# PaddlePaddle/PaddleScience

Hardware: AMD Instinct MI355X
Metric: collocation-points/sec (PDE residual+grad) (higher is better)
Workload: dtype f32

## Files before the change

include/ppsci_hip.h:

```cpp
#ifndef PPSCI_HIP_H
#define PPSCI_HIP_H

#include <stddef.h>
#include <stdint.h>

#ifdef __cplusplus
extern "C" {
#endif

#define PPSCI_MAX_IN 8
#define PPSCI_MAX_DIRS 4
#define PPSCI_MAX_OUT 8
#define PPSCI_MAX_HIDDEN 16
#define PPSCI_MAX_PROG 128
#define PPSCI_MAX_RES 8
#define PPSCI_MAX_EPARAM 8
#define PPSCI_MAX_AUX 16

enum { PPSCI_OK = 0, PPSCI_E_INVALID = -1, PPSCI_E_UNSUPPORTED = -2, PPSCI_E_LAUNCH = -3 };
enum { PPSCI_ACT_TANH = 0, PPSCI_ACT_SILU = 1, PPSCI_ACT_SIN = 2, PPSCI_ACT_SIGMOID = 3, PPSCI_ACT_COS = 4, PPSCI_ACT_GELU = 5,
       PPSCI_ACT_SWISH = 6, PPSCI_ACT_STAN = 7,
       PPSCI_ACT_RELU = 8, PPSCI_ACT_LEAKY_RELU = 9, PPSCI_ACT_ELU = 10, PPSCI_ACT_SELU = 11, PPSCI_ACT_IDENTITY = 12 };
enum { PPSCI_EMBED_NONE = 0, PPSCI_EMBED_PERIOD = 1,
       PPSCI_EMBED_STREAMS = 2 };
// ... 115 lines not shown
int ppsci_causal_weights(int64_t n_points, int n_chunks, float tol, const float* value, const float* label,
                         const float* weight, const float* area, float* chunk_scratch, float* cw, void* stream);

int ppsci_taylor_bwd(const ppsci_mlp_desc* d, const float* params, int64_t n_points,
                     const float* const* inputs_host, const float* Ubar, const void* stash,
                     void* workspace, float* grad_partials, void* stream);
int ppsci_taylor_bwd_ws(const ppsci_mlp_desc* d, const float* params, int64_t n_points,
                        const float* const* inputs_host, const float* Ubar, const void* stash,
                        void* workspace, int64_t workspace_bytes, float* grad_partials, void* stream);

typedef struct ppsci_adam_args {
  float* m;
  float* v;
  float lr, beta1, beta2, eps, grad_scale;
  int64_t step_t;
} ppsci_adam_args;

int64_t ppsci_taylor_step_workspace_bytes(const ppsci_mlp_desc* d, const ppsci_epilogue_desc* e, int64_t n_points);
int ppsci_taylor_step_kind(const ppsci_mlp_desc* d, const ppsci_epilogue_desc* e, int64_t n_points);
void ppsci_set_fused_step(int on);
void ppsci_set_step_tail(int mode);
void ppsci_set_fast_program(int on);
void ppsci_set_static_program(int on);
int ppsci_epilogue_predecode(const ppsci_epilogue_desc* e, uint32_t* out256, int* n_loads);
typedef struct ppsci_step_plan ppsci_step_plan;
ppsci_step_plan* ppsci_taylor_step_plan(const ppsci_mlp_desc* d, const ppsci_epilogue_desc* e, float* params,
                                        int64_t n_points, const float* const* inputs_host, const float* const* aux_host,
                                        float* U, float* Ubar, float* residual_out, void* stash, void* workspace,
                                        int64_t workspace_bytes, float* loss_terms, float* grad);
int ppsci_taylor_step_run(ppsci_step_plan* plan, int accumulate, const ppsci_adam_args* adam, void* stream);
#define PPSCI_STEP_KEEP_FRAGMENTS 1
int ppsci_taylor_step_run_ex(ppsci_step_plan* plan, int accumulate, const ppsci_adam_args* adam, void* stream, int flags);
int ppsci_taylor_step_plan_apply(ppsci_step_plan* plan, const ppsci_adam_args* adam, void* stream);
int ppsci_taylor_step_plan_set_scales(ppsci_step_plan* plan, const ppsci_epilogue_desc* e);
int ppsci_taylor_step_run_main(ppsci_step_plan* plan, void* stream);
void ppsci_taylor_step_plan_free(ppsci_step_plan* plan);
int ppsci_taylor_step_plan_static(const ppsci_step_plan* plan, const char** name);
int ppsci_taylor_step(const ppsci_mlp_desc* d, const ppsci_epilogue_desc* e, float* params, int64_t n_points,
                      const float* const* inputs_host, const float* const* aux_host, float* U, float* Ubar,
                      float* residual_out, void* stash, void* workspace, int64_t workspace_bytes, float* loss_terms,
                      float* grad, int accumulate, const ppsci_adam_args* adam, void* stream);

int ppsci_reduce_rows(const float* partials, int64_t rows, int64_t cols, float* out, int accumulate,
                      void* stream);

int ppsci_adam_step(int64_t n, float* params, const float* grad, float* m, float* v, float lr,
                    float beta1, float beta2, float eps, int64_t step_t, float grad_scale,
                    void* stream);

#define PPSCI_OPT_SGD 0
#define PPSCI_OPT_MOMENTUM 1
#define PPSCI_OPT_RMSPROP 2
#define PPSCI_OPT_ADAMW 3
int ppsci_optim_step(int kind, int64_t n, float* params, const float* grad, float* state1, float* state2,
                     float* state3, const float* hyper, int flag, void* stream);

int ppsci_linear_materialize(int kind, int fin, int fout, const float* v, const float* g, const float* b, float* W,
                             float* b_out, void* stream);
int ppsci_linear_pullback(int kind, int fin, int fout, const float* v, const float* g, const float* gW,
                          const float* gb, float* gv, float* gg, float* gb_out, void* stream);
// ... 256 lines not shown
```

paddlescience_amd/_lib.py:

```python
from __future__ import annotations

import ctypes as C
import os
from typing import List, Optional, Sequence

MAX_IN, MAX_DIRS, MAX_OUT, MAX_HIDDEN, MAX_PROG, MAX_RES, MAX_AUX = 8, 4, 8, 16, 128, 8, 16

ACT = {"tanh": 0, "silu": 1, "sin": 2, "sigmoid": 3, "cos": 4, "gelu": 5, "swish": 6, "stan": 7, "relu": 8, "leaky_relu": 9,
       "elu": 10, "selu": 11, "identity": 12}
PARAM_ACTS = ("swish", "stan")
SIREN_W0 = 30.0
LINEAR_PLAIN, LINEAR_WEIGHT_NORM, LINEAR_RWF, LINEAR_FOURIER, LINEAR_BROADCAST = range(5)
LINEAR_PADDED = 100
EMBED_NONE, EMBED_PERIOD, EMBED_STREAMS = 0, 1, 2

(OP_LD_IN, OP_LD_U, OP_LD_AUX, OP_CONST, OP_ADD, OP_SUB, OP_MUL, OP_DIV, OP_NEG, OP_POW, OP_SIN, OP_COS,
 OP_TANH, OP_EXP, OP_LOG, OP_SQRT, OP_ABS, OP_SINH, OP_COSH, OP_TAN, OP_MAX, OP_MIN, OP_SIGN, OP_HEAVISIDE,
 OP_DETACH, OP_ASIN, OP_ACOS, OP_ATAN, OP_ATAN2, OP_ASINH, OP_ACOSH, OP_ATANH, OP_ERF, OP_LGAMMA, OP_CEIL, OP_FLOOR,
 OP_LD_PARAM, OP_COUNT) = range(38)
MAX_EPARAM = 8
STEP_KEEP_FRAGMENTS = 1


class MlpDesc(C.Structure):
# ... 112 lines not shown
    "ppsci_epilogue_losses": (C.c_int, [C.POINTER(EpilogueDesc), C.c_int64, C.POINTER(C.c_void_p), C.c_void_p,
                                        C.POINTER(C.c_void_p), C.c_void_p, C.c_void_p, C.c_void_p, C.c_void_p,
                                        C.c_void_p, C.c_void_p, C.c_void_p, C.c_void_p]),
    "ppsci_epilogue_params": (C.c_int, [C.POINTER(EpilogueDesc), C.c_int64, C.POINTER(C.c_void_p), C.c_void_p,
                                        C.POINTER(C.c_void_p), C.c_void_p, C.c_void_p, C.c_void_p, C.c_void_p,
                                        C.c_void_p, C.c_void_p]),
    "ppsci_taylor_bwd": (C.c_int, [C.POINTER(MlpDesc), C.c_void_p, C.c_int64, C.POINTER(C.c_void_p), C.c_void_p,
                                   C.c_void_p, C.c_void_p, C.c_void_p, C.c_void_p]),
    "ppsci_taylor_bwd_ws": (C.c_int, [C.POINTER(MlpDesc), C.c_void_p, C.c_int64, C.POINTER(C.c_void_p), C.c_void_p,
                                      C.c_void_p, C.c_void_p, C.c_int64, C.c_void_p, C.c_void_p]),
    "ppsci_dense_matvec": (C.c_int, [C.c_int64, C.c_int64, C.c_void_p, C.c_void_p, C.c_void_p, C.c_float, C.c_int, C.c_void_p,
                                     C.c_void_p]),
    "ppsci_csr_matvec": (C.c_int, [C.c_int64, C.c_int64, C.c_int64, C.c_void_p, C.c_void_p, C.c_void_p, C.c_void_p, C.c_void_p,
                                   C.c_float, C.c_void_p, C.c_void_p]),
    "ppsci_reduce_rows": (C.c_int, [C.c_void_p, C.c_int64, C.c_int64, C.c_void_p, C.c_int, C.c_void_p]),
    "ppsci_taylor_step_workspace_bytes": (C.c_int64, [C.POINTER(MlpDesc), C.POINTER(EpilogueDesc), C.c_int64]),
    "ppsci_taylor_step_kind": (C.c_int, [C.POINTER(MlpDesc), C.POINTER(EpilogueDesc), C.c_int64]),
    "ppsci_set_fused_step": (None, [C.c_int]),
    "ppsci_set_step_tail": (None, [C.c_int]),
    "ppsci_set_fast_program": (None, [C.c_int]),
    "ppsci_taylor_step_run_ex": (C.c_int, [C.c_void_p, C.c_int, C.POINTER(AdamArgs), C.c_void_p, C.c_int]),
    "ppsci_taylor_step_plan_apply": (C.c_int, [C.c_void_p, C.POINTER(AdamArgs), C.c_void_p]),
    "ppsci_set_static_program": (None, [C.c_int]),
    "ppsci_epilogue_predecode": (C.c_int, [C.POINTER(EpilogueDesc), C.POINTER(C.c_uint32), C.POINTER(C.c_int)]),
    "ppsci_taylor_step_plan_static": (C.c_int, [C.c_void_p, C.POINTER(C.c_char_p)]),
    "ppsci_taylor_step_plan": (C.c_void_p, [C.POINTER(MlpDesc), C.POINTER(EpilogueDesc), C.c_void_p, C.c_int64,
                                            C.POINTER(C.c_void_p), C.POINTER(C.c_void_p), C.c_void_p, C.c_void_p, C.c_void_p,
                                            C.c_void_p, C.c_void_p, C.c_int64, C.c_void_p, C.c_void_p]),
    "ppsci_taylor_step_run": (C.c_int, [C.c_void_p, C.c_int, C.POINTER(AdamArgs), C.c_void_p]),
    "ppsci_taylor_step_plan_set_scales": (C.c_int, [C.c_void_p, C.POINTER(EpilogueDesc)]),
    "ppsci_taylor_step_run_main": (C.c_int, [C.c_void_p, C.c_void_p]),
    "ppsci_taylor_step_plan_free": (None, [C.c_void_p]),
    "ppsci_taylor_step": (C.c_int, [C.POINTER(MlpDesc), C.POINTER(EpilogueDesc), C.c_void_p, C.c_int64, C.POINTER(C.c_void_p),
                                    C.POINTER(C.c_void_p), C.c_void_p, C.c_void_p, C.c_void_p, C.c_void_p, C.c_void_p,
                                    C.c_int64, C.c_void_p, C.c_void_p, C.c_int, C.POINTER(AdamArgs), C.c_void_p]),
    "ppsci_spectral_conv2d_fwd": (C.c_int, [C.POINTER(SpectralDesc), C.c_void_p, C.c_void_p, C.c_void_p, C.c_void_p,
                                            C.c_void_p]),
    "ppsci_spectral_conv2d_bwd": (C.c_int, [C.POINTER(SpectralDesc), C.c_void_p, C.c_void_p, C.c_void_p, C.c_void_p,
                                            C.c_void_p, C.c_void_p, C.c_void_p, C.c_void_p]),
    "ppsci_spectral_conv2d_bwd_real": (C.c_int, [C.POINTER(SpectralDesc), C.c_void_p, C.c_void_p, C.c_void_p, C.c_void_p,
                                                 C.c_void_p, C.c_void_p, C.c_void_p, C.c_float, C.c_int, C.c_void_p]),
    "ppsci_spectral_conv2d_fwd_scaled": (C.c_int, [C.POINTER(SpectralDesc), C.c_void_p, C.c_void_p, C.c_void_p, C.c_void_p,
                                                   C.c_float, C.c_int, C.c_void_p]),
    "ppsci_spectral_conv2d_bwd_real_scaled": (C.c_int, [C.POINTER(SpectralDesc), C.c_void_p, C.c_void_p, C.c_void_p,
                                                        C.c_void_p, C.c_void_p, C.c_void_p, C.c_void_p, C.c_float, C.c_int,
                                                        C.c_float, C.c_int, C.c_void_p]),
# ... 206 lines not shown
```

paddlescience_amd/csrc/ppsci_common.h:

```cpp
#pragma once

#include "ppsci_hip.h"

#ifdef PPSCI_EMU
#include "hip_emu.h"
#define PPSCI_LAUNCH(KERNEL, ARGT, grid, block, lds, stream, args)                                   \
  do {                                                                                               \
    ARGT _a = (args);                                                                                \
    emu::launch_named(#KERNEL, emu_dim3{(unsigned)(grid)}, emu_dim3{(unsigned)(block)}, (size_t)(lds), \
                      [](void* p) { KERNEL(*(ARGT*)p); }, &_a);                                      \
  } while (0)
#define PPSCI_SET_MAX_LDS(KERNEL, bytes) (0)
#define PPSCI_LAST_LAUNCH_ERROR() (0)
#define PPSCI_OCCUPANCY(KERNEL, block, lds, out) (*(out) = 2, 0)
#define __builtin_amdgcn_sched_barrier(x) ((void)0)
#define ppsci_block_sync_lds() __syncthreads()
#define ppsci_block_sync_mem() __syncthreads()
#define ppsci_acquire_agent() ((void)0)
#define ppsci_setprio(p) ((void)0)
#define PPSCI_OPAQUE(v) ((void)0)
static inline void ppsci_store_agent(float* p, float v) { *p = v; }
static inline void ppsci_store_agent4(f32x4* p, f32x4 v) { *p = v; }
static inline unsigned ppsci_readlane(unsigned v, int lane) {
  float f;
  std::memcpy(&f, &v, 4);
  const float* buf = emu::wave_publish(f);
  unsigned r;
  std::memcpy(&r, &buf[lane & 63], 4);
  return r;
}
#else
#include <hip/hip_runtime.h>
typedef float f32x4 __attribute__((ext_vector_type(4)));
typedef unsigned u32x2 __attribute__((ext_vector_type(2)));
typedef unsigned u32x4 __attribute__((ext_vector_type(4)));
#define PPSCI_DYN_SMEM(name) extern __shared__ __attribute__((aligned(16))) float name[]
#define PPSCI_OPAQUE(v) asm volatile("" : "+v"(v))
__device__ __forceinline__ unsigned ppsci_cvt_pk_bf16(float a, float b) {
// ... 135 lines not shown
```

paddlescience_amd/csrc/taylor_api.hip:

```cpp
#include "taylor_tile.h"
#include "taylor_step.h"
#include "epi_static.h"

#include <math.h>
#include <stdlib.h>
#include <string.h>

#include <mutex>

__global__ void __launch_bounds__(256) ppsci_presplit_kernel(const float* params, ppsci_derived q, int H, int L, int bwd,
                                                             u32x4* out) {
  const int NB = q.NB, NKP = NB / 2;
  const int per_layer = NB * NKP * 64;
  const int total = (L - 1) * per_layer;
  for (int idx = blockIdx.x * blockDim.x + threadIdx.x; idx < total; idx += gridDim.x * blockDim.x) {
    const int l = 1 + idx / per_layer, rem = idx % per_layer;
    const int lane = rem & 63, pair = rem >> 6, rb = pair / NKP, kp = pair - rb * NKP;
    const int g = lane >> 4, c = lane & 15;
    const float* W = params + q.offW[l];
    ppsci_split4 sp[2];
#pragma unroll
    for (int hlf = 0; hlf < 2; ++hlf) {
      const int kb = 2 * kp + hlf;
      f32x4 v;
// ... 280 lines not shown
extern "C" int ppsci_taylor_bwd_ws(const ppsci_mlp_desc* d, const float* params, int64_t n_points,
                                   const float* const* inputs_host, const float* Ubar, const void* stash,
                                   void* workspace, int64_t workspace_bytes, float* grad_partials, void* stream) {
  if (workspace_bytes < 0 || n_points <= 0 || !d)
    return taylor_bwd_impl(d, params, n_points, inputs_host, Ubar, stash, workspace, grad_partials, stream);
  const int knob = ppsci_get_bwd_layerwise();
  int64_t need = ppsci_bwd_workspace_bytes(d, n_points);
  if (need > 0 && need <= workspace_bytes)
    return taylor_bwd_impl(d, params, n_points, inputs_host, Ubar, stash, workspace, grad_partials, stream);
  ppsci_set_bwd_layerwise(!knob);
  const int64_t other = ppsci_bwd_workspace_bytes(d, n_points);
  int rc;
  if (other > 0 && other <= workspace_bytes) {
    rc = taylor_bwd_impl(d, params, n_points, inputs_host, Ubar, stash, workspace, grad_partials, stream);
  } else {
    ppsci_set_error("taylor_bwd: workspace of %lld bytes, %lld needed (ppsci_bwd_workspace_bytes)", (long long)workspace_bytes,
                    (long long)need);
    rc = PPSCI_E_INVALID;
  }
  ppsci_set_bwd_layerwise(knob);
  return rc;
}

static int g_fused_step = 1, g_step_tail = -1, g_fast_vm = 1, g_static_prog = 1;
extern "C" void ppsci_set_fast_program(int on) { g_fast_vm = on ? 1 : 0; }
extern "C" void ppsci_set_static_program(int on) { g_static_prog = on ? 1 : 0; }
extern "C" int ppsci_epilogue_predecode(const ppsci_epilogue_desc* e, uint32_t* out256, int* n_loads) {
  int nl = 0;
  if (!e || !out256) return -1;
  const int n = epi_fast_encode(*e, out256, &nl);
  if (n_loads) *n_loads = nl;
  return n;
}
extern "C" void ppsci_set_fused_step(int on) { g_fused_step = on ? 1 : 0; }
extern "C" void ppsci_set_step_tail(int mode) { g_step_tail = (mode < 0 || mode > 3) ? -1 : mode; }
#define PPSCI_FUSED_TREE_MAX_GRID 48

static int run_step_act(StepArgs& a, void* stream, int launch, int* grid) {
  if (a.f.d.fourier_half > 0) return PPSCI_E_UNSUPPORTED;
  if (launch == 2 ? a.t.fused != 0 : g_fused_step != 0) {
    int rc = PPSCI_E_UNSUPPORTED;
    const bool st = a.e.static_id > 0;
    switch (a.f.d.activation) {
      case PPSCI_ACT_TANH: rc = st ? ppsci_fused_static_run_tanh(a, stream, launch, grid) : ppsci_fused_run_tanh(a, stream, launch, grid); break;
      case PPSCI_ACT_SILU: rc = st ? ppsci_fused_static_run_silu(a, stream, launch, grid) : ppsci_fused_run_silu(a, stream, launch, grid); break;
      case PPSCI_ACT_SIN: rc = st ? ppsci_fused_static_run_sin(a, stream, launch, grid) : ppsci_fused_run_sin(a, stream, launch, grid); break;
      default: break;
    }
    if (rc != PPSCI_E_UNSUPPORTED || launch == 2) return rc;
    a.e.static_id = 0;
  }
  a.t.fused = 0;
  switch (a.f.d.activation) {
    case PPSCI_ACT_TANH: return ppsci_step_run_tanh(a, stream, launch, grid);
    case PPSCI_ACT_SILU: return ppsci_step_run_silu(a, stream, launch, grid);
    case PPSCI_ACT_SIN: return ppsci_step_run_sin(a, stream, launch, grid);
    default: ppsci_set_error("taylor_step: no one-launch kernel for activation %d", a.f.d.activation); return PPSCI_E_UNSUPPORTED;
  }
}

struct StepLayout {
  long long rows_w, rows_s, rows_l, tree, counters, frag, red_tmp, red_small, red_row, fastprog, total;
  int per_tile, psmall, rowlen, tree_rows;
};
// ... 193 lines not shown
  t.rows_w = ws + y.rows_w;
  t.rows_s = ws + y.rows_s;
  t.rows_l = ws + y.rows_l;
  t.tree = ws + y.tree;
  t.counters = (unsigned*)(ws + y.counters);
  t.grad = grad;
  t.loss_terms = loss_terms;
  t.p = params;
  t.per_tile = y.per_tile;
  t.psmall = y.psmall;
  t.n_res = e->n_res;
  t.rowlen = y.rowlen;
  return plan;
}

extern "C" void ppsci_taylor_step_plan_free(ppsci_step_plan* plan) { delete plan; }

extern "C" int ppsci_taylor_step_plan_static(const ppsci_step_plan* plan, const char** name) {
  const int id = plan ? plan->a.e.static_id : 0;
  if (name) *name = epi_static_name(id);
  return id;
}

extern "C" int ppsci_taylor_step_plan_set_scales(ppsci_step_plan* plan, const ppsci_epilogue_desc* e) {
  if (!plan || !e || e->n_res != plan->a.e.e.n_res) {
    ppsci_set_error("taylor_step_plan_set_scales: invalid argument");
    return PPSCI_E_INVALID;
  }
  for (int k = 0; k < e->n_res; ++k) plan->a.e.e.res[k].scale = e->res[k].scale;
  return PPSCI_OK;
}

extern "C" int ppsci_taylor_step_run(ppsci_step_plan* plan, int accumulate, const ppsci_adam_args* adam, void* stream) {
  return ppsci_taylor_step_run_ex(plan, accumulate, adam, stream, 0);
}

extern "C" int ppsci_taylor_step_run_ex(ppsci_step_plan* plan, int accumulate, const ppsci_adam_args* adam, void* stream, int flags) {
  if (!plan) {
    ppsci_set_error("taylor_step_run: invalid argument");
    return PPSCI_E_INVALID;
  }
  StepTail& t = plan->a.t;
  t.accumulate = accumulate ? 1 : 0;
  t.do_adam = 0;
  if (adam) {
    if (!adam->m || !adam->v || adam->step_t < 1) {
// ... 140 lines not shown
```

paddlescience_amd/csrc/taylor_fused.inc:

```
#include "taylor_tile.h"
#include "taylor_step_tail.h"
#include "epi_static.h"

#include <stdlib.h>
#include <string.h>
#include <type_traits>

#ifndef PPSCI_FUSED_STATIC
#define PPSCI_FUSED_STATIC 0
#endif
#define PPSCI_FUSED_EPI_SCRATCH ((PPSCI_MAX_RES + PPSCI_MAX_EPARAM) * 16)
#define PPSCI_FUSED_MAX_IN 4
#define PPSCI_FUSED_XJ(x, j) ((j) == 0 ? (x)[0] : ((j) == 1 ? (x)[1] : ((j) == 2 ? (x)[2] : (x)[3])))

#ifdef PPSCI_FUSED_TIMERS
#define PPSCI_FT(k)                                             \
  {                                                             \
    const unsigned long long now_ = __builtin_amdgcn_s_memtime(); \
    tacc[k] += now_ - tlast;                                    \
    tlast = now_;                                               \
  }
#else
#define PPSCI_FT(k)
#endif
// ... 12 lines not shown
}

#ifdef PPSCI_DBG_DUMP
__device__ float* ppsci_dbg_buf = nullptr;
extern "C" int ppsci_dbg_set(float* p) { return (int)hipMemcpyToSymbol(HIP_SYMBOL(ppsci_dbg_buf), &p, sizeof(p)); }
#define PPSCI_DBG_STRIDE 16384
#endif


static inline long long ppsci_fused_floats(const ppsci_mlp_desc& d, const ppsci_derived& q, int S, int n_instr) {
  const int m = d.d_out, pad4m = ((m + 3) / 4) * 4;
  long long fl = 2LL * ((q.d0 + d.n_hidden + m) * q.HP + pad4m);
  fl += (q.NB + 1) * m * S * PPSCI_TILE;
  fl += q.NB * d.d_raw * PPSCI_TILE;
  fl += (long long)q.NB * m * S * PPSCI_TILE;
  fl += PPSCI_FUSED_EPI_SCRATCH + PPSCI_MAX_RES * PPSCI_TILE;
  fl += 2LL * n_instr * PPSCI_TILE;
  fl += EPI_FAST_WORDS + PPSCI_MAX_RES + PPSCI_MAX_RES * PPSCI_TILE;
  fl += 2LL * S * q.NB * 3 * 64 * 2;
  fl += PPSCI_MAX_DIRS * q.HP;
  return fl;
}

template <int NB, int LH, int N1, int N2, int ACT, bool STATIC, int ABL = 0>
__global__ void __launch_bounds__(64 * NB, 2) taylor_fused_kernel(StepArgs args) {
  constexpr int S = 1 + N1 + N2;
  constexpr int HP = 16 * NB;
  constexpr int W = NB;
  constexpr int L = LH;
  constexpr int NKP = NB / 2;
  static_assert(NB == 4, "one feature block per wave, both k-pairs of a layer's fragments held in registers");
  PPSCI_DYN_SMEM(smem);
  const FwdArgs& a = args.f;
  const int tid = threadIdx.x, nthr = blockDim.x;
  const int lane = tid & 63, wave = __builtin_amdgcn_readfirstlane(tid >> 6);
  const int g = lane >> 4, c = lane & 15;
  const int H = a.d.width, m = a.d.d_out, d0 = a.q.d0, d_raw = a.d.d_raw;
  const int pad4m = ((m + 3) / 4) * 4;
  const int n_instr = args.e.e.n_instr;

  float* W0s = smem;
  float* Bs = W0s + d0 * HP;
  float* WLs = Bs + L * HP;
  float* BLs = WLs + m * HP;
  float* gW0 = BLs + pad4m;
  float* gB = gW0 + d0 * HP;
  float* gWL = gB + L * HP;
  float* gBL = gWL + m * HP;
  float* tin = gBL + pad4m;
// ... 407 lines not shown
        }
      }
    }
    }

    fetch_x(tile + (int)gridDim.x, xr);
    PPSCI_FT(6)
    f32x4 hb[S];
#pragma unroll
    for (int s = 0; s < S; ++s) hb[s] = (f32x4){0.f, 0.f, 0.f, 0.f};
    for (int cc = 0; cc < m; ++cc) {
      float ub[S];
#pragma unroll
      for (int s = 0; s < S; ++s) ub[s] = tinw[(cc * S + s) * PPSCI_TILE + c];
      const f32x4 w4 = *(const f32x4*)&WLs[cc * HP + 16 * wave + 4 * g];
#pragma unroll
      for (int s = 0; s < S; ++s) hb[s] += w4 * ub[s];
      if (wave == 0 && !PPSCI_ABL(2)) {
        const float sb = ppsci_row_sum16_last(ub[0]);
        if (lane == 15) atomicAdd(&gBL[cc], sb);
      }
    }

    auto bwd_layer = [&](auto lc) {
      constexpr int l = decltype(lc)::value;
      const float zs = ppsci_zscale(a.d, l);
      int lanel = lane;
      PPSCI_OPAQUE(lanel);
      const int g = lanel >> 4, c = lanel & 15;
      const int xcl = ppsci_xchunk(lanel >> 4, lanel & 15);
      const int xtl = ppsci_xchunk(lanel & 3, 4 * (lanel >> 4) + ((lanel & 15) >> 2));
      const u32x4* gf = (const u32x4*)args.b.xfrag + (long long)(l > 0 ? l - 1 : 0) * PPSCI_GFRAG_PER_LAYER(NB) + lanel;
      u32x4 Ab[NKP][3];
      {
        f32x4 D1, D2, D3, hv;
        if (PPSCI_ABL(7)) {
          hv = zst[l][0];
          D1 = (f32x4){0.5f, 0.5f, 0.5f, 0.5f}, D2 = (f32x4){0.1f, 0.1f, 0.1f, 0.1f}, D3 = (f32x4){0.01f, 0.01f, 0.01f, 0.01f};
        } else
          ppsci_act_from_stash4<ACT>(zst[l][0], hv, D1, D2, D3);
#ifdef PPSCI_DBG_DUMP
        if (ppsci_dbg_buf != nullptr && l == L - 1) {
          float* q = &ppsci_dbg_buf[(long long)blockIdx.x * PPSCI_DBG_STRIDE + 5120];
          *(f32x4*)&q[(0 * 256 + tid) * 4] = D2;
          *(f32x4*)&q[(1 * 256 + tid) * 4] = D3;
        }
#endif
        if constexpr (l == L - 1) {
          f32x4 hc[S];
          hc[0] = hv;
#pragma unroll
          for (int i = 0; i < N1; ++i) {
            hc[1 + i] = D1 * zst[l][1 + i];
            if (i < N2) hc[1 + N1 + i] = D2 * zst[l][1 + i] * zst[l][1 + i] + D1 * zst[l][1 + N1 + i];
          }
          for (int cc = 0; cc < (PPSCI_ABL(2) ? 0 : m); ++cc) {
            f32x4 t = (f32x4){0.f, 0.f, 0.f, 0.f};
// ... 16 lines not shown
          *(f32x4*)&q[(2 * 256 + tid) * 4] = D1;
        }
#endif
        {
          const f32x4 two = {2.f, 2.f, 2.f, 2.f};
          f32x4 accv = D1 * hb[0];
#pragma unroll
          for (int i = 0; i < N1; ++i) {
            const f32x4 zi = zst[l][1 + i];
            const f32x4 hbi = hb[1 + i];
            f32x4 zbi = D1 * hbi;
            accv += D2 * zi * hbi;
            if (i < N2) {
              const f32x4 zii = zst[l][1 + N1 + i];
              const f32x4 hb2 = hb[1 + N1 + i];
              hb[1 + N1 + i] = D1 * hb2;
              zbi += two * D2 * zi * hb2;
              accv += (D3 * zi * zi + D2 * zii) * hb2;
            }
            hb[1 + i] = zbi;
          }
          hb[0] = accv;
        }
        if (zs != 1.f) {
#pragma unroll
          for (int s = 0; s < S; ++s) hb[s] *= zs;
        }
#ifdef PPSCI_DBG_DUMP
        if (ppsci_dbg_buf != nullptr && l == L - 1) {
#pragma unroll
          for (int s = 0; s < S; ++s) *(f32x4*)&ppsci_dbg_buf[(long long)blockIdx.x * PPSCI_DBG_STRIDE + (s * 256 + tid) * 4] = hb[s];
        }
#endif
        if (!PPSCI_ABL(2)) {
          f32x4 sb4;
#pragma unroll
          for (int r = 0; r < 4; ++r) sb4[r] = ppsci_row_sum16_last(hb[0][r]);
#ifdef PPSCI_DBG_DUMP
          if (ppsci_dbg_buf != nullptr && l == L - 1) *(f32x4*)&ppsci_dbg_buf[(long long)blockIdx.x * PPSCI_DBG_STRIDE + 4096 + tid * 4] = sb4;
#endif
          if (c == 15) {
#pragma unroll
            for (int r = 0; r < 4; ++r) atomicAdd(&gB[l * HP + 16 * wave + 4 * g + r], sb4[r]);
          }
        }
        if constexpr (l > 0) {
          __builtin_amdgcn_sched_barrier(0);
#pragma unroll
          for (int kp = 0; kp < NKP; ++kp)
#pragma unroll
            for (int q = 0; q < 3; ++q) Ab[kp][q] = gf[((wave * NKP + kp) * 3 + q) * 64];
          __builtin_amdgcn_sched_barrier(0);
#pragma unroll
          for (int s = 0; s < S; ++s) {
            const ppsci_split4 sp = ppsci_fused_split<ABL>(hb[s]);
#pragma unroll
            for (int q = 0; q < 3; ++q)
              if (!PPSCI_ABL(9) || (sp.p[q][0] == 0x12345u && sp.p[q][1] == 0x54321u)) zx[ppsci_xpair(NB, s, wave, q, xcl)] = sp.p[q];
            __builtin_amdgcn_sched_barrier(0);
          }
        }
      }

      if constexpr (l > 0) {
        __builtin_amdgcn_sched_barrier(0);
        ppsci_block_sync_lds();
        PPSCI_FT(7)
#pragma unroll
        for (int s = 0; s < S; ++s) hb[s] = (f32x4){0.f, 0.f, 0.f, 0.f};
        {
          u32x4 bq[2][S];
          const auto load_b = [&](int grp, u32x4 (&dst)[S]) {
            const int kp = grp / 3, pb = 2 - grp % 3;
#pragma unroll
            for (int s = 0; s < S; ++s) dst[s] = *(const u32x4*)&zx[ppsci_xpair(NB, s, 2 * kp, pb, xcl)];
          };
          load_b(0, bq[0]);
#pragma unroll
          for (int grp = 0; grp < 3 * NKP; ++grp) {
            const int kp = grp / 3, pb = 2 - grp % 3;
            if (grp + 1 < 3 * NKP) load_b(grp + 1, bq[(grp + 1) & 1]);
// ... 23 lines not shown
          f32x4 hcs[S];
          if (PPSCI_ABL(7)) {
            hcs[0] = zst[l - 1][0];
            E1 = (f32x4){0.5f, 0.5f, 0.5f, 0.5f}, E2 = (f32x4){0.1f, 0.1f, 0.1f, 0.1f};
          } else
            ppsci_act_from_stash4<ACT>(zst[l - 1][0], hcs[0], E1, E2, E3);
#pragma unroll
          for (int i = 0; i < N1; ++i) {
            hcs[1 + i] = E1 * zst[l - 1][1 + i];
            if (i < N2) hcs[1 + N1 + i] = E2 * zst[l - 1][1 + i] * zst[l - 1][1 + i] + E1 * zst[l - 1][1 + N1 + i];
          }
#pragma unroll
          for (int s = 0; s < S; ++s) {
            const ppsci_split4 sp = ppsci_fused_split<ABL>(hcs[s]);
#pragma unroll
            for (int q = 0; q < 3; ++q)
              if (!PPSCI_ABL(9) || (sp.p[q][0] == 0x12345u && sp.p[q][1] == 0x54321u)) hx[((s * NB + wave) * 3 + q) * 64 + xcl] = sp.p[q];
            __builtin_amdgcn_sched_barrier(0);
          }
        }
        __builtin_amdgcn_sched_barrier(0);
        if (!PPSCI_ABL(3)) ppsci_block_sync_lds();
        PPSCI_FT(9)
#pragma unroll 1
        for (int sp = 0; sp + 1 < (PPSCI_ABL(3) ? 0 : S); sp += 2) {
          int zs_ = ppsci_xpair(NB, sp, wave, 0, xtl);
          int hs_ = HPAIR ? ppsci_xpair(NB, sp, 0, 0, xtl) : xtl + sp * NB * 3 * 64;
          PPSCI_OPAQUE(zs_);
          PPSCI_OPAQUE(hs_);
          u32x2 zN0[3], zN1[3];
#pragma unroll
          for (int q = 0; q < 3; ++q) {
            zN0[q] = ppsci_lds_read_tr16(&zx[zs_ + q * 128]);
            zN1[q] = ppsci_lds_read_tr16(&zx[zs_ + (NKP * 3 + q) * 128]);
          }
          constexpr int IG = 2;
          u32x2 hN0[2][IG][3], hN1[2][IG][3];
          const auto load_h = [&](int ig, int buf) {
#pragma unroll
            for (int e = 0; e < IG; ++e)
#pragma unroll
              for (int q = 0; q < 3; ++q) {
                if constexpr (HPAIR) {
                  hN0[buf][e][q] = ppsci_lds_read_tr16(&hx[hs_ + (((ig + e) >> 1) * 3 + q) * 128 + ((ig + e) & 1)]);
                  hN1[buf][e][q] = ppsci_lds_read_tr16(&hx[hs_ + ((NKP + ((ig + e) >> 1)) * 3 + q) * 128 + ((ig + e) & 1)]);
                } else {
// ... 143 lines not shown
    const int k = idx / H, f = idx - k * H;
    ppsci_store_agent(&prow[idx], gW0[k * HP + f]);
  }
  for (int idx = tid; idx < L * H; idx += nthr) {
    const int l = idx / H, f = idx - l * H;
    ppsci_store_agent(&prow[d0 * H + idx], gB[l * HP + f]);
  }
  for (int idx = tid; idx < H * m; idx += nthr) {
    const int f = idx / m, cc = idx - f * m;
    ppsci_store_agent(&prow[(d0 + L) * H + idx], gWL[cc * HP + f]);
  }
  for (int idx = tid; idx < m; idx += nthr) ppsci_store_agent(&prow[(d0 + L + m) * H + idx], gBL[idx]);
  {
    float lsum[PPSCI_MAX_RES], padj[PPSCI_MAX_EPARAM];
#pragma unroll
    for (int k = 0; k < PPSCI_MAX_RES; ++k) lsum[k] = (wave == 0 && lane < PPSCI_TILE) ? lacc[k * PPSCI_TILE + lane] : 0.f;
#pragma unroll
    for (int k = 0; k < PPSCI_MAX_EPARAM; ++k) padj[k] = 0.f;
    epi_finale<EPI_RF_FUSED>(args.e, ered, lsum, padj);
  }
  if (args.t.external != 1) ppsci_step_tail(args.t, args.b.d, args.b.q, smem);
}

template <int NB, int LH, int N1, int N2>
static int launch_fused(StepArgs& a, void* stream, int launch, int* grid_out) {
  constexpr int S = 1 + N1 + N2;
  if (launch == 2) {
#ifdef PPSCI_ABL_BUILD
    {
      const char* ev = getenv("PPSCI_ABL");
      const int mask = ev ? atoi(ev) : 0;
#define PPSCI_ABL_CASE(M_)                                                                                                          \
  if (mask == (M_)) {                                                                                                               \
    PPSCI_SET_MAX_LDS((taylor_fused_kernel<NB, LH, N1, N2, PPSCI_ACT_ID, PPSCI_FUSED_STATIC != 0, (M_)>), a.t.lds);                    \
    PPSCI_LAUNCH((taylor_fused_kernel<NB, LH, N1, N2, PPSCI_ACT_ID, PPSCI_FUSED_STATIC != 0, (M_)>), StepArgs, a.t.grid, 64 * NB, a.t.lds, \
                 stream, a);                                                                                                        \
    return PPSCI_LAST_LAUNCH_ERROR() != 0 ? PPSCI_E_LAUNCH : PPSCI_OK;                                                              \
  }
      PPSCI_ABL_CASE(1) PPSCI_ABL_CASE(2) PPSCI_ABL_CASE(4) PPSCI_ABL_CASE(8) PPSCI_ABL_CASE(16) PPSCI_ABL_CASE(32) PPSCI_ABL_CASE(64)
      PPSCI_ABL_CASE(128) PPSCI_ABL_CASE(256) PPSCI_ABL_CASE(512)
#undef PPSCI_ABL_CASE
    }
#endif
    PPSCI_LAUNCH((taylor_fused_kernel<NB, LH, N1, N2, PPSCI_ACT_ID, PPSCI_FUSED_STATIC != 0>), StepArgs, a.t.grid, 64 * NB, a.t.lds, stream, a);
    int e = PPSCI_LAST_LAUNCH_ERROR();
    if (e != 0) {
      ppsci_set_error("taylor_fused: launch failed (hip error %d)", e);
      return PPSCI_E_LAUNCH;
    }
    return PPSCI_OK;
  }
  const long long fl = ppsci_fused_floats(a.f.d, a.f.q, S, a.e.e.n_instr);
  if (fl * 4 > PPSCI_LDS_LIMIT_BYTES / 2) {
    ppsci_set_error("taylor_fused: LDS need %lld B exceeds half a CU", fl * 4);
    return PPSCI_E_UNSUPPORTED;
  }
  const int lds = (int)(fl * 4);
  if (PPSCI_SET_MAX_LDS((taylor_fused_kernel<NB, LH, N1, N2, PPSCI_ACT_ID, PPSCI_FUSED_STATIC != 0>), lds) != 0) {
    ppsci_set_error("taylor_fused: cannot raise dynamic LDS to %d B", lds);
    return PPSCI_E_LAUNCH;
  }
  int per_cu = 1;
  if (PPSCI_OCCUPANCY((taylor_fused_kernel<NB, LH, N1, N2, PPSCI_ACT_ID, PPSCI_FUSED_STATIC != 0>), 64 * NB, lds, &per_cu) != 0 || per_cu < 1) per_cu = 1;
  const int ntl = a.f.ntiles;
  int grid = ntl < PPSCI_NUM_CU * per_cu ? ntl : PPSCI_NUM_CU * per_cu;
  if (ppsci_get_max_grid() > 0 && grid > ppsci_get_max_grid()) grid = ppsci_get_max_grid();
  if (grid < 1) grid = 1;
  a.f.iters = a.b.iters = a.e.iters = (ntl + grid - 1) / grid;
  a.f.tile0 = a.b.tile0 = 0;
  a.f.resident = a.b.resident = 1;
  a.b.accum = 1;
  a.b.xdl_split = 1;
  a.t.grid = grid;
  a.t.lds = lds;
  a.t.fused = 1;
  if (grid_out) *grid_out = grid;
  if (!launch) return PPSCI_OK;
  PPSCI_LAUNCH((taylor_fused_kernel<NB, LH, N1, N2, PPSCI_ACT_ID, PPSCI_FUSED_STATIC != 0>), StepArgs, grid, 64 * NB, lds, stream, a);
  int e = PPSCI_LAST_LAUNCH_ERROR();
  if (e != 0) {
    ppsci_set_error("taylor_fused: launch failed (hip error %d)", e);
    return PPSCI_E_LAUNCH;
  }
  return PPSCI_OK;
}

template <int N1, int N2, class... Ps>
static constexpr bool fused_has_static(epi_typelist<Ps...>) {
  return (false || ... || (Ps::N1 == N1 && Ps::N2 == N2));
}

template <int NB, int N1, int N2>
static int run_fused(StepArgs& a, void* stream, int launch, int* grid_out) {
  if constexpr (PPSCI_FUSED_STATIC != 0 && !fused_has_static<N1, N2>(EpiStaticPrograms{})) return PPSCI_E_UNSUPPORTED;
  else
  switch (a.f.d.n_hidden) {
    case 2: return launch_fused<NB, 2, N1, N2>(a, stream, launch, grid_out);
    case 3: return launch_fused<NB, 3, N1, N2>(a, stream, launch, grid_out);
    case 4: return launch_fused<NB, 4, N1, N2>(a, stream, launch, grid_out);
    case 5: return launch_fused<NB, 5, N1, N2>(a, stream, launch, grid_out);
    default: return PPSCI_E_UNSUPPORTED;
  }
}

int PPSCI_FUSED_RUN_NAME(StepArgs& a, void* stream, int launch, int* grid_out) {
#define PPSCI_FUSED_CASE(NB_, N1_, N2_) \
  if (a.f.q.NB == NB_ && a.f.d.n1 == N1_ && a.f.d.n2 == N2_ && a.f.d.n3 == 0) return run_fused<NB_, N1_, N2_>(a, stream, launch, grid_out);
// ... 10 lines not shown
```

paddlescience_amd/csrc/taylor_step.h:

```cpp
#pragma once
#include "epilogue_vm.h"

#ifdef PPSCI_EMU
#define PPSCI_STEP_FAN 3
#else
#define PPSCI_STEP_FAN 16
#endif

struct StepTail {
  float* rows_w;
  float* rows_s;
  float* rows_l;
  float* tree;
  unsigned* counters;
  float* grad;
  float* loss_terms;
  float* p;
  float* m;
  float* v;
  int grid, per_tile, psmall, n_res, rowlen;
  int lds;
  int accumulate, do_adam;
  float lr_t, beta1, beta2, eps_t, grad_scale;
  int fused;
  int one_tail;
  int external;
};

struct StepArgs {
  FwdArgs f;
  BwdArgs b;
  EpiArgs e;
  StepTail t;
};

int ppsci_step_run_tanh(StepArgs& a, void* stream, int launch, int* grid_out);
int ppsci_step_run_silu(StepArgs& a, void* stream, int launch, int* grid_out);
int ppsci_step_run_sin(StepArgs& a, void* stream, int launch, int* grid_out);
int ppsci_fused_run_tanh(StepArgs& a, void* stream, int launch, int* grid_out);
int ppsci_fused_run_silu(StepArgs& a, void* stream, int launch, int* grid_out);
int ppsci_fused_run_sin(StepArgs& a, void* stream, int launch, int* grid_out);
int ppsci_fused_static_run_tanh(StepArgs& a, void* stream, int launch, int* grid_out);
int ppsci_fused_static_run_silu(StepArgs& a, void* stream, int launch, int* grid_out);
int ppsci_fused_static_run_sin(StepArgs& a, void* stream, int launch, int* grid_out);
```

paddlescience_amd/hotpath.py:

```python
from __future__ import annotations

import ctypes as C
from dataclasses import dataclass, field
from typing import Dict, List, Optional, Sequence, Tuple

import torch

from . import _lib as L


def _stream_ptr(t: torch.Tensor):
    if t.is_cuda:
        return C.c_void_p(torch._C._cuda_getCurrentRawStream(t.device.index))
    return None


def _p(t: Optional[torch.Tensor]):
    return None if t is None else C.c_void_p(t.data_ptr())


def _chk_f32(*ts):
    for t in ts:
        if t is not None and (t.dtype != torch.float32 or not t.is_contiguous()):
            raise ValueError("hot-path buffers must be contiguous float32 tensors")
# ... 169 lines not shown
            aa = C.byref(L.AdamArgs(adam["m"].data_ptr(), adam["v"].data_ptr(), adam["lr"], adam["beta1"], adam["beta2"],
                                    adam["eps"], adam.get("grad_scale", 1.0), adam["t"]))
        capturing = self._params.is_cuda and torch.cuda.is_current_stream_capturing()
        keep = (not capturing and self._frag_token is not None
                and self._frag_token == (_PARAM_WRITES[0], self._params._version))
        L.check(self._run(self.handle, 1 if accumulate else 0, aa, _stream_ptr(self._dev), L.STEP_KEEP_FRAGMENTS if keep else 0))
        if adam is not None:
            note_param_write()
        self._frag_token = None if capturing else (_PARAM_WRITES[0], self._params._version)

    def apply_adam(self, adam: dict) -> None:
        aa = L.AdamArgs(adam["m"].data_ptr(), adam["v"].data_ptr(), adam["lr"], adam["beta1"], adam["beta2"], adam["eps"],
                        adam.get("grad_scale", 1.0), adam["t"])
        L.check(L.lib().ppsci_taylor_step_plan_apply(self.handle, C.byref(aa), _stream_ptr(self._dev)))
        note_param_write()
        capturing = self._params.is_cuda and torch.cuda.is_current_stream_capturing()
        self._frag_token = None if capturing else (_PARAM_WRITES[0], self._params._version)

    @property
    def static_program(self) -> str:
        nm = C.c_char_p()
        return (nm.value or b"").decode() if L.lib().ppsci_taylor_step_plan_static(self.handle, C.byref(nm)) > 0 else ""

    def run_main(self) -> None:
        L.check(L.lib().ppsci_taylor_step_run_main(self.handle, _stream_ptr(self._dev)))

    def __del__(self):
        h, self.handle = getattr(self, "handle", None), None
        if h:
            self._free(h)


_PARAM_WRITES = [0]


def note_param_write() -> None:
    _PARAM_WRITES[0] += 1


def dense_matvec(M: torch.Tensor, x: torch.Tensor, y: torch.Tensor, alpha: float = 1.0, transpose: bool = False,
                 rowscale: Optional[torch.Tensor] = None) -> None:
    _require_device(y)
    _chk_f32(M, x, y, rowscale)
    rows, cols = M.shape
    assert x.numel() >= (rows if transpose else cols) and y.numel() >= (cols if transpose else rows)
    L.check(L.lib().ppsci_dense_matvec(rows, cols, _p(M), _p(x), _p(rowscale), float(alpha), 1 if transpose else 0, _p(y),
# ... 181 lines not shown
```

Baseline: 445.1 million.

## Interleave next layer's pointwise adjoint with weight-gradient MFMAs in fused backward

Adds an OVL variant of the fused Taylor step kernel for static tanh programs with four streams and up to four hidden layers. In the reverse sweep, the pointwise adjoint, scaling, bias reduction, fragment load and LDS publish for layer l-1 are interleaved with the weight-gradient MFMA sweep of layer l. sched_group_barrier hints alternate matrix and VALU instructions. The aim is to hide VALU and LDS latency behind matrix-core work. The cost is higher register pressure from the carried fragment buffer, which could reduce occupancy, and a larger code footprint. It is on by default when the shape matches, with a setter and a plan query added.

```diff
diff --git a/include/ppsci_hip.h b/include/ppsci_hip.h
--- a/include/ppsci_hip.h
+++ b/include/ppsci_hip.h
@@ -161,6 +161,7 @@
 void ppsci_set_step_tail(int mode);
 void ppsci_set_fast_program(int on);
 void ppsci_set_static_program(int on);
+void ppsci_set_fused_overlap(int on);
 int ppsci_epilogue_predecode(const ppsci_epilogue_desc* e, uint32_t* out256, int* n_loads);
 typedef struct ppsci_step_plan ppsci_step_plan;
 ppsci_step_plan* ppsci_taylor_step_plan(const ppsci_mlp_desc* d, const ppsci_epilogue_desc* e, float* params,
@@ -175,6 +176,7 @@
 int ppsci_taylor_step_run_main(ppsci_step_plan* plan, void* stream);
 void ppsci_taylor_step_plan_free(ppsci_step_plan* plan);
 int ppsci_taylor_step_plan_static(const ppsci_step_plan* plan, const char** name);
+int ppsci_taylor_step_plan_overlap(const ppsci_step_plan* plan);
 int ppsci_taylor_step(const ppsci_mlp_desc* d, const ppsci_epilogue_desc* e, float* params, int64_t n_points,
                       const float* const* inputs_host, const float* const* aux_host, float* U, float* Ubar,
                       float* residual_out, void* stash, void* workspace, int64_t workspace_bytes, float* loss_terms,
diff --git a/paddlescience_amd/_lib.py b/paddlescience_amd/_lib.py
--- a/paddlescience_amd/_lib.py
+++ b/paddlescience_amd/_lib.py
@@ -158,6 +158,8 @@
     "ppsci_taylor_step_run_ex": (C.c_int, [C.c_void_p, C.c_int, C.POINTER(AdamArgs), C.c_void_p, C.c_int]),
     "ppsci_taylor_step_plan_apply": (C.c_int, [C.c_void_p, C.POINTER(AdamArgs), C.c_void_p]),
     "ppsci_set_static_program": (None, [C.c_int]),
+    "ppsci_set_fused_overlap": (None, [C.c_int]),
+    "ppsci_taylor_step_plan_overlap": (C.c_int, [C.c_void_p]),
     "ppsci_epilogue_predecode": (C.c_int, [C.POINTER(EpilogueDesc), C.POINTER(C.c_uint32), C.POINTER(C.c_int)]),
     "ppsci_taylor_step_plan_static": (C.c_int, [C.c_void_p, C.POINTER(C.c_char_p)]),
     "ppsci_taylor_step_plan": (C.c_void_p, [C.POINTER(MlpDesc), C.POINTER(EpilogueDesc), C.c_void_p, C.c_int64,
diff --git a/paddlescience_amd/csrc/ppsci_common.h b/paddlescience_amd/csrc/ppsci_common.h
--- a/paddlescience_amd/csrc/ppsci_common.h
+++ b/paddlescience_amd/csrc/ppsci_common.h
@@ -14,6 +14,7 @@
 #define PPSCI_LAST_LAUNCH_ERROR() (0)
 #define PPSCI_OCCUPANCY(KERNEL, block, lds, out) (*(out) = 2, 0)
 #define __builtin_amdgcn_sched_barrier(x) ((void)0)
+#define __builtin_amdgcn_sched_group_barrier(mask, n, id) ((void)0)
 #define ppsci_block_sync_lds() __syncthreads()
 #define ppsci_block_sync_mem() __syncthreads()
 #define ppsci_acquire_agent() ((void)0)
diff --git a/paddlescience_amd/csrc/taylor_api.hip b/paddlescience_amd/csrc/taylor_api.hip
--- a/paddlescience_amd/csrc/taylor_api.hip
+++ b/paddlescience_amd/csrc/taylor_api.hip
@@ -326,7 +326,8 @@
   return rc;
 }
 
-static int g_fused_step = 1, g_step_tail = -1, g_fast_vm = 1, g_static_prog = 1;
+static int g_fused_step = 1, g_step_tail = -1, g_fast_vm = 1, g_static_prog = 1, g_fused_overlap = 1;
+extern "C" void ppsci_set_fused_overlap(int on) { g_fused_overlap = on ? 1 : 0; }
 extern "C" void ppsci_set_fast_program(int on) { g_fast_vm = on ? 1 : 0; }
 extern "C" void ppsci_set_static_program(int on) { g_static_prog = on ? 1 : 0; }
 extern "C" int ppsci_epilogue_predecode(const ppsci_epilogue_desc* e, uint32_t* out256, int* n_loads) {
@@ -344,6 +345,7 @@
   if (a.f.d.fourier_half > 0) return PPSCI_E_UNSUPPORTED;
   if (launch == 2 ? a.t.fused != 0 : g_fused_step != 0) {
     int rc = PPSCI_E_UNSUPPORTED;
+    if (launch != 2) a.t.overlap = g_fused_overlap;
     const bool st = a.e.static_id > 0;
     switch (a.f.d.activation) {
       case PPSCI_ACT_TANH: rc = st ? ppsci_fused_static_run_tanh(a, stream, launch, grid) : ppsci_fused_run_tanh(a, stream, launch, grid); break;
@@ -583,6 +585,8 @@
   return id;
 }
 
+extern "C" int ppsci_taylor_step_plan_overlap(const ppsci_step_plan* plan) { return plan && plan->a.t.fused ? plan->a.t.overlap : 0; }
+
 extern "C" int ppsci_taylor_step_plan_set_scales(ppsci_step_plan* plan, const ppsci_epilogue_desc* e) {
   if (!plan || !e || e->n_res != plan->a.e.e.n_res) {
     ppsci_set_error("taylor_step_plan_set_scales: invalid argument");
diff --git a/paddlescience_amd/csrc/taylor_fused.inc b/paddlescience_amd/csrc/taylor_fused.inc
--- a/paddlescience_amd/csrc/taylor_fused.inc
+++ b/paddlescience_amd/csrc/taylor_fused.inc
@@ -58,9 +58,12 @@
   return fl;
 }
 
-template <int NB, int LH, int N1, int N2, int ACT, bool STATIC, int ABL = 0>
+#define PPSCI_FUSED_OVL_OK(LH_, N1_, N2_, STATIC_, ACT_) \
+  ((STATIC_) && (ACT_) == PPSCI_ACT_TANH && (N1_) == 2 && (N2_) == 1 && (LH_) <= 4)
+template <int NB, int LH, int N1, int N2, int ACT, bool STATIC, int ABL = 0, bool OVL = false>
 __global__ void __launch_bounds__(64 * NB, 2) taylor_fused_kernel(StepArgs args) {
   constexpr int S = 1 + N1 + N2;
+  static_assert(!OVL || (PPSCI_FUSED_OVL_OK(LH, N1, N2, STATIC, ACT) && ABL == 0), "the interleaved reverse sweep is written for S = 4, L <= 4");
   constexpr int HP = 16 * NB;
   constexpr int W = NB;
   constexpr int L = LH;
@@ -514,6 +517,7 @@
       }
     }
 
+    u32x4 AbT[NKP][3];
     auto bwd_layer = [&](auto lc) {
       constexpr int l = decltype(lc)::value;
       const float zs = ppsci_zscale(a.d, l);
@@ -523,8 +527,11 @@
       const int xcl = ppsci_xchunk(lanel >> 4, lanel & 15);
       const int xtl = ppsci_xchunk(lanel & 3, 4 * (lanel >> 4) + ((lanel & 15) >> 2));
       const u32x4* gf = (const u32x4*)args.b.xfrag + (long long)(l > 0 ? l - 1 : 0) * PPSCI_GFRAG_PER_LAYER(NB) + lanel;
-      u32x4 Ab[NKP][3];
-      {
+      constexpr bool PW_DONE = OVL && l < L - 1;
+      u32x4 AbL[NKP][3];
+      u32x4(&Ab)[NKP][3] = *(PW_DONE ? &AbT : &AbL);
+      const auto pw_adjoint = [&](auto kc) {
+        constexpr int l = decltype(kc)::value;
         f32x4 D1, D2, D3, hv;
         if (PPSCI_ABL(7)) {
           hv = zst[l][0];
@@ -587,6 +594,9 @@
           }
           hb[0] = accv;
         }
+      };
+      const auto pw_scale = [&](auto kc, const float zs) {
+        constexpr int l = decltype(kc)::value;
         if (zs != 1.f) {
 #pragma unroll
           for (int s = 0; s < S; ++s) hb[s] *= zs;
@@ -597,31 +607,47 @@
           for (int s = 0; s < S; ++s) *(f32x4*)&ppsci_dbg_buf[(long long)blockIdx.x * PPSCI_DBG_STRIDE + (s * 256 + tid) * 4] = hb[s];
         }
 #endif
-        if (!PPSCI_ABL(2)) {
-          f32x4 sb4;
-#pragma unroll
-          for (int r = 0; r < 4; ++r) sb4[r] = ppsci_row_sum16_last(hb[0][r]);
+      };
+      const auto pw_bias_sum = [&](auto kc) {
+        constexpr int l = decltype(kc)::value;
+        f32x4 sb4;
+#pragma unroll
+        for (int r = 0; r < 4; ++r) sb4[r] = ppsci_row_sum16_last(hb[0][r]);
 #ifdef PPSCI_DBG_DUMP
-          if (ppsci_dbg_buf != nullptr && l == L - 1) *(f32x4*)&ppsci_dbg_buf[(long long)blockIdx.x * PPSCI_DBG_STRIDE + 4096 + tid * 4] = sb4;
-#endif
-          if (c == 15) {
-#pragma unroll
-            for (int r = 0; r < 4; ++r) atomicAdd(&gB[l * HP + 16 * wave + 4 * g + r], sb4[r]);
-          }
-        }
+        if (ppsci_dbg_buf != nullptr && l == L - 1) *(f32x4*)&ppsci_dbg_buf[(long long)blockIdx.x * PPSCI_DBG_STRIDE + 4096 + tid * 4] = sb4;
+#endif
+        return sb4;
+      };
+      const auto pw_bias_add = [&](auto kc, const f32x4 sb4) {
+        constexpr int l = decltype(kc)::value;
+        if (c == 15) {
+#pragma unroll
+          for (int r = 0; r < 4; ++r) atomicAdd(&gB[l * HP + 16 * wave + 4 * g + r], sb4[r]);
+        }
+      };
+      const auto pw_frag = [&](const u32x4* gf, u32x4(&dst)[NKP][3]) {
+#pragma unroll
+        for (int kp = 0; kp < NKP; ++kp)
+#pragma unroll
+          for (int q = 0; q < 3; ++q) dst[kp][q] = gf[((wave * NKP + kp) * 3 + q) * 64];
+      };
+      const auto pw_publish = [&](int s) {
+        const ppsci_split4 sp = ppsci_fused_split<ABL>(hb[s]);
+#pragma unroll
+        for (int q = 0; q < 3; ++q)
+          if (!PPSCI_ABL(9) || (sp.p[q][0] == 0x12345u && sp.p[q][1] == 0x54321u)) zx[ppsci_xpair(NB, s, wave, q, xcl)] = sp.p[q];
+      };
+      if constexpr (!PW_DONE) {
+        pw_adjoint(lc);
+        pw_scale(lc, zs);
+        if (!PPSCI_ABL(2)) pw_bias_add(lc, pw_bias_sum(lc));
         if constexpr (l > 0) {
           __builtin_amdgcn_sched_barrier(0);
-#pragma unroll
-          for (int kp = 0; kp < NKP; ++kp)
-#pragma unroll
-            for (int q = 0; q < 3; ++q) Ab[kp][q] = gf[((wave * NKP + kp) * 3 + q) * 64];
+          pw_frag(gf, Ab);
           __builtin_amdgcn_sched_barrier(0);
 #pragma unroll
           for (int s = 0; s < S; ++s) {
-            const ppsci_split4 sp = ppsci_fused_split<ABL>(hb[s]);
-#pragma unroll
-            for (int q = 0; q < 3; ++q)
-              if (!PPSCI_ABL(9) || (sp.p[q][0] == 0x12345u && sp.p[q][1] == 0x54321u)) zx[ppsci_xpair(NB, s, wave, q, xcl)] = sp.p[q];
+            pw_publish(s);
             __builtin_amdgcn_sched_barrier(0);
           }
         }
@@ -691,6 +717,65 @@
         __builtin_amdgcn_sched_barrier(0);
         if (!PPSCI_ABL(3)) ppsci_block_sync_lds();
         PPSCI_FT(9)
+        if constexpr (OVL) {
+          constexpr std::integral_constant<int, l - 1> kc{};
+          const auto wbar_pair = [&](auto spc, auto&& filler) {
+            constexpr int sp = decltype(spc)::value;
+            constexpr int NV = 4;
+            int zs_ = ppsci_xpair(NB, sp, wave, 0, xtl);
+            int hs_ = HPAIR ? ppsci_xpair(NB, sp, 0, 0, xtl) : xtl + sp * NB * 3 * 64;
+            PPSCI_OPAQUE(zs_);
+            PPSCI_OPAQUE(hs_);
+            __builtin_amdgcn_sched_barrier(0);
+            u32x2 zN0[3], zN1[3], hN0[NB][3], hN1[NB][3];
+#pragma unroll
+            for (int q = 0; q < 3; ++q) {
+              zN0[q] = ppsci_lds_read_tr16(&zx[zs_ + q * 128]);
+              zN1[q] = ppsci_lds_read_tr16(&zx[zs_ + (NKP * 3 + q) * 128]);
+            }
+#pragma unroll
+            for (int e = 0; e < NB; ++e)
+#pragma unroll
+              for (int q = 0; q < 3; ++q) {
+                if constexpr (HPAIR) {
+                  hN0[e][q] = ppsci_lds_read_tr16(&hx[hs_ + ((e >> 1) * 3 + q) * 128 + (e & 1)]);
+                  hN1[e][q] = ppsci_lds_read_tr16(&hx[hs_ + ((NKP + (e >> 1)) * 3 + q) * 128 + (e & 1)]);
+                } else {
+                  hN0[e][q] = ppsci_lds_read_tr16(&hx[hs_ + (e * 3 + q) * 64]);
+                  hN1[e][q] = ppsci_lds_read_tr16(&hx[hs_ + ((NB + e) * 3 + q) * 64]);
+                }
+              }
+            filler();
+            constexpr int IG = 2;
+#pragma unroll
+            for (int ig = 0; ig < NB; ig += IG)
+#pragma unroll
+              for (int q = 0; q < PPSCI_XDL_NPROD; ++q)
+#pragma unroll
+                for (int e = 0; e < IG; ++e)
+                  wacc[l - 1][ig + e] = ppsci_xdl32(hN0[ig + e][ppsci_xdl_pa[q]], hN1[ig + e][ppsci_xdl_pa[q]], zN0[ppsci_xdl_pb[q]],
+                                                    zN1[ppsci_xdl_pb[q]], wacc[l - 1][ig + e]);
+#pragma unroll
+            for (int i = 0; i < NB * PPSCI_XDL_NPROD; ++i) {
+              __builtin_amdgcn_sched_group_barrier(0x8, 1, 0);
+              __builtin_amdgcn_sched_group_barrier(0x2, NV, 0);
+            }
+            __builtin_amdgcn_sched_barrier(0);
+          };
+          static_assert(S == 4, "two stream pairs: region A, region B");
+          wbar_pair(std::integral_constant<int, 0>{}, [&]() { pw_adjoint(kc); });
+          pw_scale(kc, ppsci_zscale(a.d, l - 1));
+          f32x4 sb4 = {0.f, 0.f, 0.f, 0.f};
+          wbar_pair(std::integral_constant<int, 2>{}, [&]() {
+            sb4 = pw_bias_sum(kc);
+            if constexpr (l > 1) {
+              pw_frag((const u32x4*)args.b.xfrag + (long long)(l - 2) * PPSCI_GFRAG_PER_LAYER(NB) + lanel, AbT);
+#pragma unroll
+              for (int s = 0; s < S; ++s) pw_publish(s);
+            }
+          });
+          pw_bias_add(kc, sb4);
+        } else
 #pragma unroll 1
         for (int sp = 0; sp + 1 < (PPSCI_ABL(3) ? 0 : S); sp += 2) {
           int zs_ = ppsci_xpair(NB, sp, wave, 0, xtl);
@@ -880,8 +965,8 @@
   if (args.t.external != 1) ppsci_step_tail(args.t, args.b.d, args.b.q, smem);
 }
 
-template <int NB, int LH, int N1, int N2>
-static int launch_fused(StepArgs& a, void* stream, int launch, int* grid_out) {
+template <int NB, int LH, int N1, int N2, bool OVL>
+static int launch_fused_k(StepArgs& a, void* stream, int launch, int* grid_out) {
   constexpr int S = 1 + N1 + N2;
   if (launch == 2) {
 #ifdef PPSCI_ABL_BUILD
@@ -900,7 +985,7 @@
 #undef PPSCI_ABL_CASE
     }
 #endif
-    PPSCI_LAUNCH((taylor_fused_kernel<NB, LH, N1, N2, PPSCI_ACT_ID, PPSCI_FUSED_STATIC != 0>), StepArgs, a.t.grid, 64 * NB, a.t.lds, stream, a);
+    PPSCI_LAUNCH((taylor_fused_kernel<NB, LH, N1, N2, PPSCI_ACT_ID, PPSCI_FUSED_STATIC != 0, 0, OVL>), StepArgs, a.t.grid, 64 * NB, a.t.lds, stream, a);
     int e = PPSCI_LAST_LAUNCH_ERROR();
     if (e != 0) {
       ppsci_set_error("taylor_fused: launch failed (hip error %d)", e);
@@ -914,12 +999,12 @@
     return PPSCI_E_UNSUPPORTED;
   }
   const int lds = (int)(fl * 4);
-  if (PPSCI_SET_MAX_LDS((taylor_fused_kernel<NB, LH, N1, N2, PPSCI_ACT_ID, PPSCI_FUSED_STATIC != 0>), lds) != 0) {
+  if (PPSCI_SET_MAX_LDS((taylor_fused_kernel<NB, LH, N1, N2, PPSCI_ACT_ID, PPSCI_FUSED_STATIC != 0, 0, OVL>), lds) != 0) {
     ppsci_set_error("taylor_fused: cannot raise dynamic LDS to %d B", lds);
     return PPSCI_E_LAUNCH;
   }
   int per_cu = 1;
-  if (PPSCI_OCCUPANCY((taylor_fused_kernel<NB, LH, N1, N2, PPSCI_ACT_ID, PPSCI_FUSED_STATIC != 0>), 64 * NB, lds, &per_cu) != 0 || per_cu < 1) per_cu = 1;
+  if (PPSCI_OCCUPANCY((taylor_fused_kernel<NB, LH, N1, N2, PPSCI_ACT_ID, PPSCI_FUSED_STATIC != 0, 0, OVL>), 64 * NB, lds, &per_cu) != 0 || per_cu < 1) per_cu = 1;
   const int ntl = a.f.ntiles;
   int grid = ntl < PPSCI_NUM_CU * per_cu ? ntl : PPSCI_NUM_CU * per_cu;
   if (ppsci_get_max_grid() > 0 && grid > ppsci_get_max_grid()) grid = ppsci_get_max_grid();
@@ -934,13 +1019,24 @@
   a.t.fused = 1;
   if (grid_out) *grid_out = grid;
   if (!launch) return PPSCI_OK;
-  PPSCI_LAUNCH((taylor_fused_kernel<NB, LH, N1, N2, PPSCI_ACT_ID, PPSCI_FUSED_STATIC != 0>), StepArgs, grid, 64 * NB, lds, stream, a);
+  PPSCI_LAUNCH((taylor_fused_kernel<NB, LH, N1, N2, PPSCI_ACT_ID, PPSCI_FUSED_STATIC != 0, 0, OVL>), StepArgs, grid, 64 * NB, lds, stream, a);
   int e = PPSCI_LAST_LAUNCH_ERROR();
   if (e != 0) {
     ppsci_set_error("taylor_fused: launch failed (hip error %d)", e);
     return PPSCI_E_LAUNCH;
   }
   return PPSCI_OK;
+}
+
+template <int NB, int LH, int N1, int N2>
+static int launch_fused(StepArgs& a, void* stream, int launch, int* grid_out) {
+#ifndef PPSCI_ABL_BUILD
+  if constexpr (PPSCI_FUSED_OVL_OK(LH, N1, N2, PPSCI_FUSED_STATIC != 0, PPSCI_ACT_ID)) {
+    if (a.t.overlap) return launch_fused_k<NB, LH, N1, N2, true>(a, stream, launch, grid_out);
+  }
+#endif
+  a.t.overlap = 0;
+  return launch_fused_k<NB, LH, N1, N2, false>(a, stream, launch, grid_out);
 }
 
 template <int N1, int N2, class... Ps>
diff --git a/paddlescience_amd/csrc/taylor_step.h b/paddlescience_amd/csrc/taylor_step.h
--- a/paddlescience_amd/csrc/taylor_step.h
+++ b/paddlescience_amd/csrc/taylor_step.h
@@ -25,6 +25,7 @@
   int fused;
   int one_tail;
   int external;
+  int overlap;
 };
 
 struct StepArgs {
diff --git a/paddlescience_amd/hotpath.py b/paddlescience_amd/hotpath.py
--- a/paddlescience_amd/hotpath.py
+++ b/paddlescience_amd/hotpath.py
@@ -215,6 +215,10 @@
         nm = C.c_char_p()
         return (nm.value or b"").decode() if L.lib().ppsci_taylor_step_plan_static(self.handle, C.byref(nm)) > 0 else ""
 
+    @property
+    def overlap(self) -> bool:
+        return L.lib().ppsci_taylor_step_plan_overlap(self.handle) == 1
+
     def run_main(self) -> None:
         L.check(L.lib().ppsci_taylor_step_run_main(self.handle, _stream_ptr(self._dev)))
 
```

Measured after the change: 456.5 million (median of 6 runs). 1.03x the previous value.
